# BlueFern/CRDModel

Measured on AMD Instinct MI355X. Metric: grid-point-steps/sec, FHN torus 8192x8192 RK4, higher is better.
Workload: dtype f64

## Files before the change

### crdmodel_amd/__init__.py

```python
from . import _capi
from ._capi import CrdError
from .solver import (Ensemble, LocalGroup, PinnedArray, Recorder, Slab, Writer, block_extents, cycle_agreed, cycle_vote, dims_create, grid_of, halo_plan, initial_conditions, kernel_digest, kernel_digest_of_table_row, kernel_table_digest, launch_plan_candidates, load_ini, make_params, plan_key, rccl_unique_id,
                     run_config, slab_extents, stable_dt, steady_state, steady_state_as_printed)
```

### crdmodel_amd/_capi.py

```python
import ctypes as C
import importlib.util
import os
import sys

_PKG = os.path.dirname(os.path.abspath(__file__))
LIB_PATH = os.environ.get("CRD_LIBRARY") or os.path.join(_PKG, "libcrd.so")

ABI_VERSION = 8
OK, EINVAL, ENOMEM, EHIP, ERCCL, EIO, EPARSE, ESTATE = 0, -1, -2, -3, -4, -5, -6, -7
MODEL_FHN, MODEL_GOLDBETER = 0, 1
SURFACE_TORUS, SURFACE_FLAT = 0, 1
PRECISION_F64, PRECISION_F32 = 0, 1
STEPPER_AUTO, STEPPER_STAGED, STEPPER_FUSED = 0, 1, 2
ADAPT_RK43, ADAPT_ARKODE = 0, 1

MODELS = {"fhn": MODEL_FHN, "goldbeter": MODEL_GOLDBETER}
SURFACES = {"torus": SURFACE_TORUS, "flat": SURFACE_FLAT}
STEPPERS = {"auto": STEPPER_AUTO, "staged": STEPPER_STAGED, "fused": STEPPER_FUSED}


class Params(C.Structure):

    _fields_ = [
        ("model", C.c_int32), ("surface", C.c_int32),
# ... 154 lines not shown
    "crd_dominant_kernel_name": (C.c_char_p, [_vp]),
    "crd_state_max_abs": (C.c_int, [_vp, C.POINTER(C.c_double)]),
    "crd_trace_range_push": (None, [C.c_char_p]),
    "crd_trace_range_pop": (None, []),
    "crd_set_autotune": (C.c_int, [_vp, C.c_int]),
    "crd_get_launch_plan": (C.c_int, [_vp, C.POINTER(LaunchPlan)]),
    "crd_get_launch_geometry": (C.c_int, [_vp, C.POINTER(LaunchGeometry)]),
    "crd_set_launch_plan": (C.c_int, [_vp, C.c_int, C.c_int, C.c_int, C.c_int, C.c_int]),
    "crd_plan_launches": (C.c_int, [_vp]),
    "crd_set_diagnostics": (C.c_int, [_vp, C.c_int]),
    "crd_set_halo_slack": (C.c_int, [_vp, C.c_int]),
    "crd_set_exchange_period": (C.c_int, [_vp, C.c_int]),
    "crd_get_exchange_period": (C.c_int, [_vp]),
    "crd_group_set_threads": (C.c_int, [C.POINTER(_vp), C.c_int, C.c_int]),
    "crd_launch_plan_candidate": (C.c_int, [C.c_int, C.POINTER(LaunchPlan)]),
    "crd_get_step_timing": (C.c_int, [_vp, C.POINTER(StepTiming)]),
    "crd_ensemble_create": (C.c_int, [C.POINTER(Params), C.c_int, C.c_int, C.POINTER(_vp)]),
    "crd_ensemble_create_mixed": (C.c_int, [C.POINTER(Params), C.c_int, C.c_int, C.POINTER(_vp)]),
    "crd_ensemble_member_grid": (C.c_int, [_vp, C.c_int, C.POINTER(Grid)]),
    "crd_ensemble_destroy": (None, [_vp]),
    "crd_ensemble_last_error": (C.c_char_p, [_vp]),
    "crd_ensemble_info": (C.c_int, [_vp, C.POINTER(C.c_int), C.POINTER(Grid)]),
    "crd_ensemble_upload": (C.c_int, [_vp, C.c_int, _vp, C.c_int]),
    "crd_ensemble_download": (C.c_int, [_vp, C.c_int, _vp, C.c_int]),
    "crd_ensemble_step_rk4": (C.c_int, [_vp, C.c_double, C.c_double, C.c_int64]),
    "crd_ensemble_step_rk4_own": (C.c_int, [_vp, C.c_double, C.c_double, C.POINTER(C.c_int64)]),
    "crd_ensemble_step_rk4_own_dt": (C.c_int, [_vp, C.c_double, C.c_double, C.POINTER(C.c_double), C.POINTER(C.c_int64)]),
    "crd_ensemble_step_rk4_own_timed": (C.c_int, [_vp, C.c_double, C.c_double, C.POINTER(C.c_int64), C.POINTER(C.c_double)]),
    "crd_ensemble_own_steps": (C.c_int, [_vp, C.c_double, C.c_double, C.c_double, C.POINTER(C.c_int64)]),
    "crd_ensemble_step_rk4_timed": (C.c_int, [_vp, C.c_double, C.c_double, C.c_int64, C.POINTER(C.c_double)]),
# ... 82 lines not shown
```

### crdmodel_amd/csrc/crd_context.cpp

```cpp
#include <algorithm>
#include <cmath>
#include <cstdio>
#include <cstdlib>
#include <cstring>
#include <new>

#include "crd_ctx.h"
#include "crd_ensemble.h"
#include "crd_tuning.h"

namespace crd {

namespace {
thread_local std::string g_create_error;
}

int fail(crd_ctx *c, int code, const std::string &msg)
{
	if (c) c->err = msg; else g_create_error = msg;
	return code;
}

int set_device(crd_ctx *c)
{
// ... 723 lines not shown
	hipDeviceProp_t prop;
	HIP_TRY(c, hipGetDeviceProperties(&prop, c->device));
	out->simds = 4 * prop.multiProcessorCount;
	out->clock_khz = prop.clockRate;
	return CRD_OK;
}

int crd_launch_plan_candidate(int index, crd_launch_plan *out)
{
	if (!out) return CRD_EINVAL;
	*out = crd_launch_plan{};
	if (!fused_plan_candidate(index, &out->one_round, &out->xcd_mapping, &out->columns_per_lane, &out->nontemporal_stores, &out->steps_per_launch)) return CRD_EINVAL;
	return CRD_OK;
}

int crd_state_max_abs(crd_ctx *c, double *out)
{
	if (!c || !out) return CRD_EINVAL;
	if (int rc = set_device(c)) return rc;
	double *sink = c->scalar_sink();
	HIP_TRY(c, launch_max_abs(c->p.precision, c->plane[crd_ctx::Y][0], c->nx, c->nyl, sink, c->compute));
	if (sink != c->scalar_host) HIP_TRY(c, hipMemcpyAsync(c->scalar_host, sink, sizeof(double), hipMemcpyDeviceToHost, c->compute));
	HIP_TRY(c, hipStreamSynchronize(c->compute));
	*out = c->scalar_host[0];
	return CRD_OK;
}

int crd_state_observe(crd_ctx *c, double stats[8])
{
	if (!c || !stats) return CRD_EINVAL;
// ... 57 lines not shown
```

### crdmodel_amd/csrc/crd_fused.hip

```cpp
#include "crd_fused_impl.h"

namespace crd {

bool fused_step_supported(int, const SlabDesc &d) { return d.nyl >= 2 * kStepHalo; }

bool fused_two_steps_supported(const SlabDesc &d) { return d.nyl >= 4 * kStepHalo && kernel_model(d) != kModelDiffusionOnly; }

int fused_steps_supported(int precision, const SlabDesc &d, int want)
{
	bool three = kernel_model(d) == CRD_MODEL_FHN && (precision == CRD_PRECISION_F64 || d.nx % 2 == 0);
#ifdef CRD_THREE_STEPS_GOLDBETER
	three = three || (precision == CRD_PRECISION_F64 && kernel_model(d) == CRD_MODEL_GOLDBETER);
#endif
	if (want >= 3 && three && (d.wrap || precision != CRD_PRECISION_F64) && d.nyl >= 6 * kStepHalo) return 3;
	return (want >= 2 && fused_two_steps_supported(d)) ? 2 : 1;
}

bool fused_wide_supported(int precision, const SlabDesc &d, int want_steps)
{
	return precision == CRD_PRECISION_F64 && kernel_model(d) == CRD_MODEL_FHN && fused_steps_supported(precision, d, want_steps) == 3;
}

int fused_max_items(const SlabDesc &d)
{
	const int strips = (d.nx + (kValid - 2) - 1) / (kValid - 2);
	return strips * ((d.nyl + 2 * kGhost + 3) / 4 + 2);
}

const char *fused_kernel_name(int, int) { return "crd_rk4_fused_step_kernel"; }

int fused_default_columns(int precision, int nx) { return (precision == CRD_PRECISION_F32 && nx % 2 == 0) ? 2 : 1; }
// ... 37 lines not shown
```

### crdmodel_amd/csrc/crd_fused_impl.h

```cpp
#pragma once
#include <hip/hip_runtime.h>
#include <hip/hip_ext.h>

#include <algorithm>
#include <cstdint>
#include <cstdio>
#include <cstdlib>
#include <type_traits>
#include <utility>

#include "crd_device.h"
#include "crd_tuning.h"

namespace crd {

namespace {

using namespace dev;

constexpr int kApron = 4;
constexpr int kLanes = 64;
constexpr int kValid = kLanes - 2 * kApron;
constexpr int kWavesPerBlock = 4;
constexpr int kMaxWavesPerBlock = 4;
// ... 81 lines not shown
template <typename Real, int MODEL, int COLS, int STEPS = 2>
constexpr bool kCoop = sizeof(Real) == 8 && COLS == 1;
#elif defined(CRD_NO_COOP)
template <typename Real, int MODEL, int COLS, int STEPS = 2>
constexpr bool kCoop = false;
#else
template <typename Real, int MODEL, int COLS, int STEPS = 2>
constexpr bool kCoop = sizeof(Real) == 8 && COLS == 1 && (MODEL == CRD_MODEL_GOLDBETER || STEPS == 3);
#endif
#if defined(CRD_NO_READ_AHEAD)
template <typename Real, int MODEL, int COLS, int STEPS>
constexpr bool kReadAhead = false;
#else
template <typename Real, int MODEL, int COLS, int STEPS>
constexpr bool kReadAhead = kCoop<Real, MODEL, COLS, STEPS> && STEPS == 3;
#endif
constexpr int kWideWaves = 8;
template <typename Real, int MODEL, int COLS, int STEPS>
constexpr bool kCanWide = sizeof(Real) == 8 && MODEL == CRD_MODEL_FHN && COLS == 1 && STEPS == 3 && kCoop<Real, MODEL, COLS, STEPS>;
template <int STEPS>
constexpr int kEdgeSlotBytes = STEPS == 3 ? 128 : 64;
template <int STEPS, int WAVES = 4 >
constexpr int kEdgeParityBytes = WAVES * 2 * kEdgeSlotBytes<STEPS>;
template <int STEPS, int WAVES = 4>
constexpr int kEdgeBytes = 2 * kEdgeParityBytes<STEPS, WAVES>;
template <int STEPS, int WAVES = 4>
constexpr int kEdgeDumpBytes = WAVES * 64 * 8 + kEdgeBytes<STEPS, WAVES>;
__device__ __forceinline__ double from_lane_below_old(double x, double old)
{
	int lo = __double2loint(x), hi = __double2hiint(x);
// ... 355 lines not shown
constexpr int kRingRowsWanted = CRD_RING_ROWS;
#ifndef CRD_RING_ROWS_THREE
#define CRD_RING_ROWS_THREE 8
#endif
template <typename V, int STEPS = 2>
constexpr int kRingRowsOf = (kLanes * (int)sizeof(V) / 256 >= 4 && (STEPS == 3 ? CRD_RING_ROWS_THREE : kRingRowsWanted) > 4) ? 4 : (STEPS == 3 ? CRD_RING_ROWS_THREE : kRingRowsWanted);
typedef unsigned int u32x2 __attribute__((ext_vector_type(2)));
typedef unsigned int u32x4 __attribute__((ext_vector_type(4)));
typedef __attribute__((address_space(3))) char lds_char;
constexpr unsigned kRowResourceBytes = 0x7fffffffu;
constexpr unsigned kStoreNowhere = 0x80000000u;
__device__ __forceinline__ __amdgpu_buffer_rsrc_t row_resource(const void *row)
{
	return __builtin_amdgcn_make_buffer_rsrc(const_cast<void *>(row), 0, (int)kRowResourceBytes, 0x00020000);
}
template <bool NT, typename V>
__device__ __forceinline__ void buffer_row_store(__amdgpu_buffer_rsrc_t r, unsigned byte_offset, V v)
{
	constexpr int aux = NT ? 2 : 0;
	if constexpr (sizeof(V) == 4) __builtin_amdgcn_raw_buffer_store_b32(__builtin_bit_cast(unsigned, v), r, byte_offset, 0, aux);
	else if constexpr (sizeof(V) == 8) __builtin_amdgcn_raw_buffer_store_b64(__builtin_bit_cast(u32x2, v), r, byte_offset, 0, aux);
	else __builtin_amdgcn_raw_buffer_store_b128(__builtin_bit_cast(u32x4, v), r, byte_offset, 0, aux);
}
template <int VMCNT, int OFF_U, int OFF_V, typename V>
__device__ __forceinline__ void ring_read(unsigned lds_lane, V &u, V &v)
{
	if constexpr (sizeof(V) == 4)
		asm volatile("s_waitcnt vmcnt(%3)\n\tds_read_b32 %0, %2 offset:%4\n\tds_read_b32 %1, %2 offset:%5\n\ts_waitcnt lgkmcnt(0)"
		             : "=&v"(u), "=&v"(v) : "v"(lds_lane), "n"(VMCNT), "n"(OFF_U), "n"(OFF_V) : "memory");
	else if constexpr (sizeof(V) == 8)
		asm volatile("s_waitcnt vmcnt(%3)\n\tds_read_b64 %0, %2 offset:%4\n\tds_read_b64 %1, %2 offset:%5\n\ts_waitcnt lgkmcnt(0)"
		             : "=&v"(u), "=&v"(v) : "v"(lds_lane), "n"(VMCNT), "n"(OFF_U), "n"(OFF_V) : "memory");
	else
		asm volatile("s_waitcnt vmcnt(%3)\n\tds_read_b128 %0, %2 offset:%4\n\tds_read_b128 %1, %2 offset:%5\n\ts_waitcnt lgkmcnt(0)"
		             : "=&v"(u), "=&v"(v) : "v"(lds_lane), "n"(VMCNT), "n"(OFF_U), "n"(OFF_V) : "memory");
}
template <int VMCNT, int OFF_U, int OFF_V>
// ... 58 lines not shown
#endif
#endif
	using V = typename LaneValue<Real, COLS>::type;
	constexpr int APRON = STEPS * kApron;
	constexpr int FILL = 2 * APRON;
	static_assert(APRON % COLS == 0, "the apron is whole lanes");
	constexpr int VALID = COLS * kLanes - 2 * APRON;
	constexpr int M = 4;
	constexpr int RB = kLanes * (int)sizeof(V), SLOT = 2 * RB, G1 = RB / 256, kRingRows = kRingRowsOf<V, STEPS>;
	static_assert(kRingRows % M == 0 && kRingRows >= M && (kRingRows & (kRingRows - 1)) == 0, "ring slots are addressed with the unrolled iteration index");
	constexpr int kWaitFill = (kRingRows - 1) * 2 * G1, kWaitSteady = kWaitFill + 2 * kRingRows;
	static_assert(kWaitSteady <= 63, "vmcnt is six bits");
	constexpr bool AHEAD = kReadAhead<Real, MODEL, COLS, STEPS>;
	constexpr int kWaitAhead = kWaitFill + 2 * (kRingRows - 1);
	static_assert(kWaitAhead <= 63, "vmcnt is six bits");
	const int lane = threadIdx.x & (kLanes - 1);
	const int nx = s.nx;
	const int wave = __builtin_amdgcn_readfirstlane((int)(threadIdx.x >> 6));
	const int x0 = COOP ? sblk * (a.sw * kLanes - 2 * APRON) - APRON + wave * kLanes : strip * VALID - APRON;
	const int place = COOP ? wave * kLanes + lane : COLS * lane, span = COOP ? a.sw * kLanes : COLS * kLanes;
	int x = x0 + COLS * lane;
	x %= nx;
	if (x < 0) x += nx;
	const unsigned xb = (unsigned)x * (unsigned)sizeof(Real);
	const int out_col = x0 + COLS * lane;
	const bool lane_stores = place >= APRON && place < span - APRON && out_col < nx;
	const unsigned xb_store = lane_stores ? xb : kStoreNowhere;

	const int range = chunk >= a.first2 ? 1 : 0;
	const int range_end = a.r_end[range];
// ... 1 lines not shown
	const int j1 = (j0 + a.chunk < range_end) ? j0 + a.chunk : range_end;
	const int jbase = j0 - APRON;
	const int niter = (j1 - j0) + 2 * APRON;
	const int jlast = j1 + APRON - 1;

	const V cE = *reinterpret_cast<const V *>(s.cE + x), cWn = *reinterpret_cast<const V *>(s.cWn + x), cP = *reinterpret_cast<const V *>(s.cP + x);
	const Real ka4 = s.ka4;
	const V h1 = (V)a.h1, h2 = (V)a.h2, h3 = (V)a.h3, h6 = (V)a.h6;
	const __attribute__((address_space(4))) Real *const brow = (const __attribute__((address_space(4))) Real *)(s.brow);
	const int wrap_nyl = s.wrap ? s.nyl : 0;
	auto row_base = [&](int j) -> ptrdiff_t {
		j += wrap_nyl & (j >> 31);
		j -= (j >= s.nyl) ? wrap_nyl : 0;
		return (ptrdiff_t)j * nx;
	};
	int jb = 0, amask = 0;
	if (ABSORB) {
		int g0 = (a.js + jbase) % a.ny;
		if (g0 < 0) g0 += a.ny;
		jb = jbase + (a.ny - 1 - g0);
#pragma unroll
		for (int k = 0; k < 4; k++) amask |= (a.absorb[k] ? 1 << k : 0) | (a.absorb2[k] ? 16 << k : 0) | ((STEPS == 3 && a.absorb3[k]) ? 256 << k : 0);
		jb = __builtin_amdgcn_readfirstlane(jb);
		amask = __builtin_amdgcn_readfirstlane(amask);
	}
	const int ny_rows = a.ny;
	auto boundary_row = [&](int j) -> bool { return (unsigned)(j - jb) <= 1u || (unsigned)(j - jb - ny_rows) <= 1u; };

	struct Pipe {
		V u0[M], v0[M], U1[M], U2[M], U3[M], V1[2], V2[2], V3[2], aU[M], aV[M];
// ... 16 lines not shown
	if constexpr (COOP) {
		const unsigned base = (unsigned)(uintptr_t)block_edges;
		edge_pub = (lane == 0 || lane == kLanes - 1) ? base + (unsigned)((wave * 2 + (lane == 0 ? 0 : 1)) * kEdgeSlotBytes<STEPS>)
		                                             : base + (unsigned)(kEdgeBytes<STEPS, WAVES> + (wave * kLanes + lane) * 8);
		edge_con = base + (unsigned)((lane == 0 ? (wave > 0 ? wave - 1 : wave) * 2 + 1 : (wave + 1 < a.sw ? wave + 1 : wave) * 2) * kEdgeSlotBytes<STEPS>);
	}
	const unsigned ring_lane = (unsigned)(uintptr_t)ring + (unsigned)lane * (unsigned)sizeof(V);
	unsigned doff[G1];
#pragma unroll
	for (int h = 0; h < G1; h++) {
		const int q = 4 * (kLanes * h + lane), e = q / (int)sizeof(Real);
		int col = (x0 + e) % nx;
		if (col < 0) col += nx;
		doff[h] = (unsigned)col * (unsigned)sizeof(Real) + (unsigned)(q % (int)sizeof(Real));
	}
	auto fill = [&](int jrow, int slot_byte) {
		const ptrdiff_t rb = row_base(jrow);
		const __amdgpu_buffer_rsrc_t ru = row_resource(a.in_u + rb), rv = row_resource(a.in_v + rb);
#pragma unroll
		for (int h = 0; h < G1; h++) __builtin_amdgcn_raw_ptr_buffer_load_lds(ru, ring + (slot_byte + 256 * h), 4, doff[h], 0, 0, 0);
#pragma unroll
		for (int h = 0; h < G1; h++) __builtin_amdgcn_raw_ptr_buffer_load_lds(rv, ring + (slot_byte + RB + 256 * h), 4, doff[h], 0, 0, 0);
	};
#pragma unroll
	for (int k = 0; k < kRingRows; k++) fill((jbase + k < jlast) ? jbase + k : jlast, k * SLOT);
	int jn = (jbase + kRingRows < jlast) ? jbase + kRingRows : jlast;
	if constexpr (AHEAD) ring_read_ahead<kWaitFill, 0, RB>(ring_lane, P[0].u0[0], P[0].v0[0]);
	Real pb = brow[jbase];
	int trip_byte = 0;
	unsigned ring_trip = ring_lane;
	Real *out_row_u = a.out_u + (ptrdiff_t)(jbase - APRON) * nx, *out_row_v = a.out_v + (ptrdiff_t)(jbase - APRON) * nx;
	if constexpr (AHEAD) ring_first_row_landed(P[0].u0[0], P[0].v0[0]);

	[[maybe_unused]] double2r edge[2 * STEPS];
#pragma unroll
	for (int q = 0; q < 2 * STEPS; q++) edge[q] = double2r{0.0, 0.0};
	auto point = [&](V uC, V uS, V uN, V v, Real rowp, bool zero, [[maybe_unused]] V X, V &du, V &dv) {
		if constexpr (COOP) rhs_lane_edge<MODEL>(uC, X, uS, uN, v, cE, cWn, cP, rowp, ka4, zero, du, dv);
		else rhs_lane<V, MODEL>(uC, uS, uN, v, cE, cWn, cP, rowp, ka4, zero, du, dv);
	};
	auto stages = [&](Pipe &Q, const int p, auto kk, auto live_c, const int flag_bit, const Real b4, V &nu, V &nv, [[maybe_unused]] const V (&E)[4], auto qbase_c) {
// ... 27 lines not shown
			Q.aV[S3] = stage_fma(h3, dv, Q.aV[S3]);
		}
		nu = nv = zero_v;
		if constexpr (live >= 8) {
			point(Q.U3[S4], Q.U3[S5], Q.U3[S3], Q.V3[S4 & 1], b4, ABSORB && ((amask >> (flag_bit + 3)) & 1) && boundary_row(p - 4), E[3], du, dv);
			nu = stage_fma(h6, du, Q.aU[S4]);
			nv = stage_fma(h6, dv, Q.aV[S4]);
		}
	};
	auto next_trip = [&]() {
		if constexpr (kRingRows > M) {
			trip_byte = (trip_byte + M * SLOT) & (kRingRows * SLOT - 1);
			ring_trip = ring_lane + (unsigned)trip_byte;
		}
	};
	auto iteration = [&](int m, auto kk, auto fed_c) {
		constexpr int FED = decltype(fed_c)::value;
		constexpr int K = decltype(kk)::value;
		constexpr int S0 = K % M, S4 = (K + 2 * M - 4) % M;
#if !defined(CRD_NO_LOCKSTEP) && !defined(CRD_NO_LOCKSTEP_TWO)
		if constexpr (sizeof(Real) == 4 && STEPS == 2) __builtin_amdgcn_s_barrier();
#endif
		const int p = jbase + m;
		Real b4[STEPS];
#pragma unroll
		for (int n = 0; n < STEPS; n++) b4[n] = P[n].bq[S4];
		if (!AHEAD && m < FILL + kRingRows) asm volatile("s_waitcnt vmcnt(%0)" ::"n"(kWaitFill) : "memory");
		V E[STEPS][4];
		auto take_row = [&]() {
			P[0].bq[S0] = uniform(pb);
#ifndef CRD_PROBE_NOLOAD
			fill(jn, trip_byte + S0 * SLOT);
#endif
			jn = (jn < jlast) ? jn + 1 : jlast;
		};
		if constexpr (AHEAD) {
			edge_publish<(K & 1) * kEdgeParityBytes<STEPS, WAVES>>(edge_pub, P[0].u0[S0]);
			take_row();
			if constexpr (K == M - 1) next_trip();
			ring_row_landed(edge);
			pb = brow[(p < jlast) ? p + 1 : jlast];
#pragma unroll
			for (int n = 0; n < STEPS; n++) E[n][0] = edge[2 * n].x, E[n][1] = edge[2 * n].y, E[n][2] = edge[2 * n + 1].x, E[n][3] = edge[2 * n + 1].y;
		} else if constexpr (COOP) {
			ring_read_with_edges<kWaitSteady, S0 * SLOT, S0 * SLOT + RB>(ring_trip, P[0].u0[S0], P[0].v0[S0], edge);
#pragma unroll
			for (int n = 0; n < STEPS; n++) E[n][0] = edge[2 * n].x, E[n][1] = edge[2 * n].y, E[n][2] = edge[2 * n + 1].x, E[n][3] = edge[2 * n + 1].y;
			edge_publish<(K & 1) * kEdgeParityBytes<STEPS, WAVES>>(edge_pub, P[0].u0[S0]);
		} else {
			ring_read<kWaitSteady, S0 * SLOT, S0 * SLOT + RB>(ring_trip, P[0].u0[S0], P[0].v0[S0]);
#pragma unroll
			for (int n = 0; n < STEPS; n++) E[n][0] = E[n][1] = E[n][2] = E[n][3] = zero_v;
		}
		if constexpr (!AHEAD) {
			take_row();
			pb = brow[(p < jlast) ? p + 1 : jlast];
		}
		V nu, nv;
		if constexpr (PRIO) __builtin_amdgcn_s_setprio(0);
		[[maybe_unused]] auto read_ahead = [&]() {
			if (m + 1 < FILL + kRingRows) asm volatile("s_waitcnt vmcnt(%0)" ::"n"(kWaitFill) : "memory");
			ring_read_ahead<kWaitAhead, ((K + 1) % M) * SLOT, ((K + 1) % M) * SLOT + RB>(ring_trip, P[0].u0[(K + 1) % M], P[0].v0[(K + 1) % M]);
		};
#ifdef CRD_PROBE_NOMATH
		nu = P[0].u0[S0] + (V)b4[0];
		nv = P[0].v0[S0] + (V)b4[STEPS - 1];
		if constexpr (AHEAD) read_ahead();
#else
		for_sequence(
		    [&](auto nn) {
			    constexpr int N = decltype(nn)::value;
#ifdef CRD_PROBE_HALFMATH
			    if constexpr (N > 0) return;
#endif
			    if constexpr (N > 0) {
				    P[N].u0[S0] = nu;
				    P[N].v0[S0] = nv;
				    P[N].bq[S0] = b4[N - 1];
				    if constexpr (COOP) edge_publish<(K & 1) * kEdgeParityBytes<STEPS, WAVES> + 32 * N>(edge_pub, nu);
			    }
			    constexpr int live = FED - 8 * N < 0 ? 0 : (FED - 8 * N > 8 ? 8 : FED - 8 * N);
			    stages(P[N], p - kApron * N, kk, std::integral_constant<int, live>{}, 4 * N, b4[N], nu, nv, E[N], std::integral_constant<int, 4 * N>{});
			    if constexpr (AHEAD && N == 0) read_ahead();
		    },
		    std::make_integer_sequence<int, STEPS>{});
#endif
		if constexpr (PRIO) __builtin_amdgcn_s_setprio(2);
		if constexpr (FED >= FILL) {
#if defined(CRD_PROBE_BRANCHY_STORES)
			if (lane_stores) {
				buffer_row_store<NT>(row_resource(out_row_u), xb, nu);
				buffer_row_store<NT>(row_resource(out_row_v), xb, nv);
			}
#elif !defined(CRD_PROBE_NOSTORE)
			buffer_row_store<NT>(row_resource(out_row_u), xb_store, nu);
			buffer_row_store<NT>(row_resource(out_row_v), xb_store, nv);
#else
			if (a.nchunks < 0) {
				buffer_row_store<NT>(row_resource(out_row_u), xb_store, nu);
				buffer_row_store<NT>(row_resource(out_row_v), xb_store, nv);
			}
#endif
		}
		out_row_u += nx;
		out_row_v += nx;
		if constexpr (AHEAD) edge_exchange<(K & 1) * kEdgeParityBytes<STEPS, WAVES>>(edge_con, edge, P[0].u0[(K + 1) % M], P[0].v0[(K + 1) % M]);
		else if constexpr (COOP) edge_exchange<(K & 1) * kEdgeParityBytes<STEPS, WAVES>>(edge_con, edge);
	};
	int m = 0;
	for_sequence(
	    [&](auto i) {
		    constexpr int I = decltype(i)::value;
		    iteration(I, std::integral_constant<int, I % M>{}, i);
		    if constexpr (!AHEAD && I % M == M - 1) next_trip();
	    },
	    std::make_integer_sequence<int, FILL>{});
	m = FILL;
	for (; m + M - 1 < niter; m += M) {
		for_sequence([&](auto k) { iteration(m + decltype(k)::value, k, std::integral_constant<int, FILL>{}); }, std::make_integer_sequence<int, M>{});
		if constexpr (!AHEAD) next_trip();
	}
	for_sequence(
	    [&](auto k) {
		    if (m + decltype(k)::value < niter) iteration(m + decltype(k)::value, k, std::integral_constant<int, FILL>{});
	    },
	    std::make_integer_sequence<int, M - 1>{});
	if constexpr (AHEAD)
		asm volatile("s_waitcnt vmcnt(0) lgkmcnt(0)"
		             : "+v"(P[0].u0[0]), "+v"(P[0].u0[1]), "+v"(P[0].u0[2]), "+v"(P[0].u0[3]), "+v"(P[0].v0[0]), "+v"(P[0].v0[1]), "+v"(P[0].v0[2]), "+v"(P[0].v0[3])
		             :
		             : "memory");
	else asm volatile("s_waitcnt vmcnt(0)" ::: "memory");
}

template <typename Real, int MODEL, int COLS, int STEPS, bool ABSORB>
constexpr int kMinWaves = (STEPS == 2 && COLS * (int)sizeof(Real) == 8 && MODEL == CRD_MODEL_FHN && !ABSORB) ? 3 : (STEPS == 3 ? 2 : 1);
template <typename Real, int MODEL, bool ABSORB, int EMBED, int COLS, bool NT = false, int STEPS = 1, int WAVES = kMaxWavesPerBlock>
__global__ void __launch_bounds__(kLanes *WAVES) __attribute__((amdgpu_waves_per_eu(kMinWaves<Real, MODEL, COLS, STEPS, ABSORB>))) crd_rk4_fused_step_kernel(Slab<Real> s, FusedArgs<Real> a)
{
// ... 157 lines not shown
hipError_t launch_fused_t(const SlabDesc &d, const FusedCall &c, int row_begin, int row_end, int row_begin2, int row_end2, int js, int ny,
                          hipStream_t st)
{
	clear_launch_status();
	if (row_end <= row_begin) {
		if (c.geometry) return hipSuccess;
		if (c.start_event)
			if (hipError_t e = hipEventRecord(c.start_event, st); e != hipSuccess) return e;
		if (c.done_event)
			if (hipError_t e = hipEventRecord(c.done_event, st); e != hipSuccess) return e;
		return hipSuccess;
	}
	if (row_end2 < row_begin2) row_end2 = row_begin2;
	constexpr bool kCanTwoSteps = MODEL != kModelDiffusionOnly;
	if (c.steps != 1 && (c.embed || !((c.steps == 2 && kCanTwoSteps) || (c.steps == 3 && kCanThreeSteps<Real, MODEL> && (kThreeStepCols<Real, MODEL> == 1 || d.nx % 2 == 0)))))
		return hipErrorInvalidValue;
	if (!d.wrap && (row_begin < -(kGhost - c.steps * kStepHalo) || row_end > d.nyl + (kGhost - c.steps * kStepHalo))) return hipErrorInvalidValue;
	const Slab<Real> s = typed<Real>(d);
	FusedArgs<Real> a;
	a.in_u = row0<Real>(c.y0.u, d.nx);
	a.in_v = row0<Real>(c.y0.v, d.nx);
	a.out_u = row0<Real>(c.yout.u, d.nx);
	a.out_v = row0<Real>(c.yout.v, d.nx);
	a.h2 = (Real)(0.5 * c.dt);
	a.h3 = (Real)(c.dt / 3.0);
	a.h6 = (Real)(c.dt / 6.0);
	a.h1 = (Real)c.dt;
	for (int k = 0; k < 5; k++) a.absorb[k] = c.absorb[k];
	for (int k = 0; k < 4; k++) a.absorb2[k] = c.absorb2[k];
	for (int k = 0; k < 4; k++) a.absorb3[k] = c.absorb3[k];
// ... 220 lines not shown
				else set_io(c.yout, c.tune_scratch);
				flip ^= 1;
			}
			return fire();
		};
		if (pingpong && err == hipSuccess) {
			configure(0, 0, cols_default, 0);
			err = fire();
		}
		constexpr int kCandidates = kNumPlanCandidates, kRounds = 3;
		const bool room_for_two = d.wrap || (row_begin >= -(kGhost - 2 * kStepHalo) && row_end <= d.nyl + (kGhost - 2 * kStepHalo));
		const bool two_steps_ok = kCanTwoSteps && !c.embed && c.steps == 1 && d.nyl >= 4 * kStepHalo && room_for_two;
		const bool room_for_three = d.wrap || (row_begin >= -(kGhost - 3 * kStepHalo) && row_end <= d.nyl + (kGhost - 3 * kStepHalo));
		const bool three_steps_ok = two_steps_ok && kCanThreeSteps<Real, MODEL> && (kThreeStepCols<Real, MODEL> == 1 || cols2_ok) && d.nyl >= 6 * kStepHalo &&
		                            (d.wrap || sizeof(Real) == 4) && room_for_three &&
		                            !(sizeof(Real) == 4 && absorb12);
		float t_best[kCandidates];
		bool live[kCandidates];
		int reps = 3;
		for (int k = 0; k < kCandidates; k++) {
			t_best[k] = 0.f;
			configure(kPlanCandidates[k].one_round, kPlanCandidates[k].remap, kPlanCandidates[k].cols, kPlanCandidates[k].nt, kPlanCandidates[k].steps);
			live[k] = k == 0 || !(kPlanCandidates[k].one_round && a.chunk == fused_chunk_rows<Real, MODEL>(a.nstrips, rows, 0, cols, steps));
			if (live[k] && kPlanCandidates[k].one_round != plan_mode) live[k] = false;
			if (live[k] && kPlanCandidates[k].steps != ((kPlanCandidates[k].steps == 3 ? three_steps_ok : two_steps_ok) ? steps : 1)) live[k] = false;
			if (live[k] && steps == 2 && cols == 2 && sizeof(Real) == 8) live[k] = false;
			if (live[k] && kPlanCandidates[k].remap != a.remap) live[k] = false;
			if (live[k] && kPlanCandidates[k].cols != cols) live[k] = false;
			if (live[k] && (kPlanCandidates[k].nt != 0) != nt) live[k] = false;
		}
// ... 112 lines not shown
```

### crdmodel_amd/csrc/crd_kernels.h

```cpp
#pragma once

#include <hip/hip_runtime.h>

#include <cstdint>

namespace crd {

struct Planes {
	void *u;
	void *v;
};

struct SlabDesc {
	const void *cE;
	const void *cWn;
	const void *cP;
	const void *brow;
	double ka4;
	int nx;
	int nyl;
	int wrap;
	int wrap_x = 1;
	int has_row0;
	int has_rowN;
// ... 67 lines not shown
	FusedGeometry *geometry = nullptr;
	hipEvent_t done_event = nullptr;
	hipEvent_t start_event = nullptr;
};
hipError_t launch_fused_step(int precision, const SlabDesc &d, const FusedCall &c, int row_begin, int row_end, int row_begin2, int row_end2,
                             hipStream_t s);
hipError_t launch_sum_partials(const double *partials, int n, double *out, hipEvent_t done, hipStream_t s);
const char *fused_kernel_name(int precision, int model);
bool fused_step_supported(int precision, const SlabDesc &d);
int fused_default_columns(int precision, int nx);
int fused_plan_candidates();
bool fused_plan_candidate(int index, int *chunk_mode, int *mapping, int *cols, int *nt, int *steps);
bool fused_two_steps_supported(const SlabDesc &d);
bool fused_wide_supported(int precision, const SlabDesc &d, int want_steps);
int fused_steps_supported(int precision, const SlabDesc &d, int want);
int fused_max_items(const SlabDesc &d);

hipError_t launch_aos_to_planes(int precision, int src_is_f64, const void *aos, Planes dst, int nx, int nyl, hipStream_t s);
hipError_t launch_planes_to_aos(int precision, int dst_is_f64, Planes src, void *aos, int nx, int nyl, hipStream_t s);
hipError_t launch_aos_row_extract(int precision, const void *aos, void *row, int nx, int j, hipStream_t s);
hipError_t launch_aos_cols_extract(int precision, const void *aos, void *col_w, void *col_e, int nx, int nyl, hipStream_t s);
hipError_t launch_plane_cols_extract(int precision, const void *u_plane, void *col_w, void *col_e, int nx, int nyl, hipStream_t s);

hipError_t launch_hermite(int precision, Planes yn, Planes yp, Planes fn, Planes fp, Planes out, int nx, int nyl, double theta, double h, hipStream_t s);

hipError_t launch_hin_bound(int precision, Planes y, Planes f, int nx, int nyl, double rtol, double atol, double *out_dev, hipStream_t s);
hipError_t launch_axpy_planes(int precision, Planes y, Planes f, double h, Planes out, int nx, int nyl, hipStream_t s);
hipError_t launch_ydd_sumsq(int precision, Planes y, Planes f0, Planes f2, double h, double rtol, double atol, int nx, int nyl, double *partials_dev, double *out_dev,
                            hipStream_t s);

// ... 6 lines not shown
```

### crdmodel_amd/solver.py

```python
import ctypes as C

import numpy as np

from . import _capi as capi
from .post import period_map
from ._capi import (MODELS, SURFACES, STEPPERS, PRECISION_F32, PRECISION_F64, CrdError, Grid, Params,
                    RunConfig, check, lib)


def make_params(model, surface, nx, surface_length, surface_width, diffusion, beta, *, ny=0, beta_min=0.0, beta_max=0.0,
                vary_beta=0, just_diffusion=0, t_boundary=0.0, precision="f64"):
    p = Params()
    p.model = MODELS[model] if isinstance(model, str) else model
    p.surface = SURFACES[surface] if isinstance(surface, str) else surface
    p.nx, p.ny = nx, ny
    p.surface_length, p.surface_width = surface_length, surface_width
    p.diffusion, p.beta, p.beta_min, p.beta_max = diffusion, beta, beta_min, beta_max
    p.vary_beta, p.just_diffusion = vary_beta, just_diffusion
    p.t_boundary = t_boundary
    p.precision = {"f64": PRECISION_F64, "f32": PRECISION_F32}[precision] if isinstance(precision, str) else precision
    return p


def grid_of(params):
# ... 556 lines not shown
        except Exception:
            pass


def launch_plan_candidates(eight_wide=False):
    out, k = [], 0
    while True:
        lp = capi.LaunchPlan()
        if lib().crd_launch_plan_candidate(k, C.byref(lp)) != 0:
            return out
        if (lp.one_round == 3) == bool(eight_wide):
            out.append((lp.one_round, lp.xcd_mapping, lp.columns_per_lane, lp.nontemporal_stores, lp.steps_per_launch))
        k += 1


def plan_key(model, precision, plan):
    if isinstance(plan, dict):
        plan = (plan["one_round"], plan["xcd_mapping"], plan["columns_per_lane"], plan["nontemporal_stores"], plan.get("steps_per_launch", 1))
    key = "fused/%s/%s/chunk%d/map%d/cols%d/%s" % (model, precision, plan[0], plan[1], plan[2], "nt" if plan[3] else "plain")
    return key + ("/steps%d" % plan[4] if len(plan) > 4 and plan[4] >= 2 else "")


def kernel_table_digest():
    return lib().crd_kernel_table_digest().decode()


def kernel_digest(geometry):
    import hashlib

    fields = ("vgprs", "sgprs", "lds_bytes", "scratch_bytes", "wavefronts_per_simd", "loop_valu", "loop_salu", "loop_vmem", "loop_lds", "loop_instructions", "exec_skipped_vmem")
# ... 188 lines not shown
```

### include/crd.h

```cpp
#ifndef CRD_H
#define CRD_H

#include <stddef.h>
#include <stdint.h>

#ifdef __cplusplus
extern "C" {
#endif

#define CRD_ABI_VERSION 8

typedef enum crd_status {
	CRD_OK = 0,
	CRD_EINVAL = -1,
	CRD_ENOMEM = -2,
	CRD_EHIP = -3,
	CRD_ERCCL = -4,
	CRD_EIO = -5,
	CRD_EPARSE = -6,
	CRD_ESTATE = -7
} crd_status;

enum { CRD_MODEL_FHN = 0, CRD_MODEL_GOLDBETER = 1 };
enum { CRD_SURFACE_TORUS = 0, CRD_SURFACE_FLAT = 1 };
// ... 221 lines not shown
	int32_t rows;
	int32_t strips, chunk_rows, chunks;
	int32_t workgroups, wavefronts_per_workgroup;
	int32_t fill_iterations;
	int32_t iterations_per_trip;
	int32_t lanes, lanes_valid;
	int32_t vgprs, sgprs, lds_bytes, scratch_bytes, wavefronts_per_simd;
	int32_t loop_valu, loop_salu, loop_vmem, loop_lds, loop_instructions;
	int32_t simds, clock_khz;
	int32_t exec_skipped_vmem;
	int64_t wavefront_iterations;
	int64_t wavefront_iterations_effective;
} crd_launch_geometry;
int crd_get_launch_geometry(crd_ctx *ctx, crd_launch_geometry *out);
int crd_launch_plan_candidate(int index, crd_launch_plan *out);
int crd_set_launch_plan(crd_ctx *ctx, int chunk_mode, int xcd_mapping, int columns_per_lane, int nontemporal_stores, int steps_per_launch);
int crd_plan_launches(crd_ctx *ctx);

void crd_trace_range_push(const char *name);
void crd_trace_range_pop(void);

int crd_state_max_abs(crd_ctx *ctx, double *out);

typedef struct crd_ensemble crd_ensemble;
int crd_ensemble_create(const crd_params *members, int n_members, int device, crd_ensemble **out);
int crd_ensemble_create_mixed(const crd_params *members, int n_members, int device, crd_ensemble **out);
void crd_ensemble_destroy(crd_ensemble *e);
const char *crd_ensemble_last_error(const crd_ensemble *e);
int crd_ensemble_info(const crd_ensemble *e, int *n_members, crd_grid *g);
int crd_ensemble_member_grid(const crd_ensemble *e, int member, crd_grid *g);
// ... 68 lines not shown
```

Measured before the change: 352.4 billion.

## Address fused three-step rows via scalar offsets on fixed buffer resources

In the read-ahead three-step fused kernel, per-row buffer resource construction for loads and stores is replaced. Four buffer resources are built once per slab, and a scalar row byte offset (soffset) is advanced each row, with a torus seam wrap. The steady-state loop is also peeled from the ring-fill phase so the conditional vmcnt wait drops out of the main loop. The aim is to cut scalar/vector address arithmetic and resource setup in the inner loop. A 32-bit addressability guard, with new C/Python query helpers, falls back to fewer steps per launch when a slab exceeds 4 GiB.

After: 358.7 billion, median of 6. +1.8%, better.

```diff
diff --git a/crdmodel_amd/__init__.py b/crdmodel_amd/__init__.py
--- a/crdmodel_amd/__init__.py
+++ b/crdmodel_amd/__init__.py
@@ -1,4 +1,4 @@
 from . import _capi
 from ._capi import CrdError
 from .solver import (Ensemble, LocalGroup, PinnedArray, Recorder, Slab, Writer, block_extents, cycle_agreed, cycle_vote, dims_create, grid_of, halo_plan, initial_conditions, kernel_digest, kernel_digest_of_table_row, kernel_table_digest, launch_plan_candidates, load_ini, make_params, plan_key, rccl_unique_id,
-                     run_config, slab_extents, stable_dt, steady_state, steady_state_as_printed)
+                     rows_addressable, run_config, slab_extents, stable_dt, steady_state, steady_state_as_printed, steps_per_launch_on)
diff --git a/crdmodel_amd/_capi.py b/crdmodel_amd/_capi.py
--- a/crdmodel_amd/_capi.py
+++ b/crdmodel_amd/_capi.py
@@ -192,6 +192,8 @@
     "crd_get_exchange_period": (C.c_int, [_vp]),
     "crd_group_set_threads": (C.c_int, [C.POINTER(_vp), C.c_int, C.c_int]),
     "crd_launch_plan_candidate": (C.c_int, [C.c_int, C.POINTER(LaunchPlan)]),
+    "crd_steps_per_launch_on": (C.c_int, [C.c_int, C.c_int, C.c_int64, C.c_int64, C.c_int, C.c_int]),
+    "crd_rows_addressable": (C.c_int, [C.c_int64, C.c_int64, C.c_int]),
     "crd_get_step_timing": (C.c_int, [_vp, C.POINTER(StepTiming)]),
     "crd_ensemble_create": (C.c_int, [C.POINTER(Params), C.c_int, C.c_int, C.POINTER(_vp)]),
     "crd_ensemble_create_mixed": (C.c_int, [C.POINTER(Params), C.c_int, C.c_int, C.POINTER(_vp)]),
diff --git a/crdmodel_amd/csrc/crd_context.cpp b/crdmodel_amd/csrc/crd_context.cpp
--- a/crdmodel_amd/csrc/crd_context.cpp
+++ b/crdmodel_amd/csrc/crd_context.cpp
@@ -761,6 +761,26 @@
 	return CRD_OK;
 }
 
+int crd_rows_addressable(int64_t nx, int64_t rows, int real_bytes)
+{
+	if (nx > INT32_MAX || rows > INT32_MAX) return 0;
+	return fused_scalar_rows_addressable((long)nx, (long)rows, (long)real_bytes) ? 1 : 0;
+}
+
+int crd_steps_per_launch_on(int model, int precision, int64_t nx, int64_t nyl, int single_slab, int steps_wanted)
+{
+	if ((model != CRD_MODEL_FHN && model != CRD_MODEL_GOLDBETER) || (precision != CRD_PRECISION_F64 && precision != CRD_PRECISION_F32) || nx < 1 || nyl < 1 || nx > INT32_MAX ||
+	    nyl > INT32_MAX || steps_wanted < 1 || steps_wanted > 3)
+		return CRD_EINVAL;
+	SlabDesc d{};
+	d.nx = (int)nx;
+	d.nyl = (int)nyl;
+	d.ny = (int)nyl;
+	d.wrap = single_slab ? 1 : 0;
+	d.model = model;
+	return fused_steps_supported(precision, d, steps_wanted);
+}
+
 int crd_state_max_abs(crd_ctx *c, double *out)
 {
 	if (!c || !out) return CRD_EINVAL;
diff --git a/crdmodel_amd/csrc/crd_fused.hip b/crdmodel_amd/csrc/crd_fused.hip
--- a/crdmodel_amd/csrc/crd_fused.hip
+++ b/crdmodel_amd/csrc/crd_fused.hip
@@ -12,9 +12,12 @@
 #ifdef CRD_THREE_STEPS_GOLDBETER
 	three = three || (precision == CRD_PRECISION_F64 && kernel_model(d) == CRD_MODEL_GOLDBETER);
 #endif
+	if (precision == CRD_PRECISION_F64 && !fused_scalar_rows_addressable(d.nx, fused_addressed_rows(d), 8)) three = false;
 	if (want >= 3 && three && (d.wrap || precision != CRD_PRECISION_F64) && d.nyl >= 6 * kStepHalo) return 3;
 	return (want >= 2 && fused_two_steps_supported(d)) ? 2 : 1;
 }
+
+long fused_addressed_rows(const SlabDesc &d) { return (long)d.nyl + (d.wrap ? 0L : 2L * kGhost); }
 
 bool fused_wide_supported(int precision, const SlabDesc &d, int want_steps)
 {
diff --git a/crdmodel_amd/csrc/crd_fused_impl.h b/crdmodel_amd/csrc/crd_fused_impl.h
--- a/crdmodel_amd/csrc/crd_fused_impl.h
+++ b/crdmodel_amd/csrc/crd_fused_impl.h
@@ -119,6 +119,13 @@
 #else
 template <typename Real, int MODEL, int COLS, int STEPS>
 constexpr bool kReadAhead = kCoop<Real, MODEL, COLS, STEPS> && STEPS == 3;
+#endif
+#if defined(CRD_NO_SCALAR_ROWS)
+template <typename Real, int MODEL, int COLS, int STEPS>
+constexpr bool kScalarRows = false;
+#else
+template <typename Real, int MODEL, int COLS, int STEPS>
+constexpr bool kScalarRows = kReadAhead<Real, MODEL, COLS, STEPS>;
 #endif
 constexpr int kWideWaves = 8;
 template <typename Real, int MODEL, int COLS, int STEPS>
@@ -504,13 +511,23 @@
 {
 	return __builtin_amdgcn_make_buffer_rsrc(const_cast<void *>(row), 0, (int)kRowResourceBytes, 0x00020000);
 }
+template <bool ON>
+struct ScalarRows {
+};
+template <>
+struct ScalarRows<true> {
+	__amdgpu_buffer_rsrc_t in_u, in_v, out_u, out_v;
+	unsigned pitch, seam, in_off, out_off, b_off, b_last;
+	int row_lo;
+	const __attribute__((address_space(4))) char *b_first;
+};
 template <bool NT, typename V>
-__device__ __forceinline__ void buffer_row_store(__amdgpu_buffer_rsrc_t r, unsigned byte_offset, V v)
+__device__ __forceinline__ void buffer_row_store(__amdgpu_buffer_rsrc_t r, unsigned byte_offset, V v, unsigned row_offset = 0)
 {
 	constexpr int aux = NT ? 2 : 0;
-	if constexpr (sizeof(V) == 4) __builtin_amdgcn_raw_buffer_store_b32(__builtin_bit_cast(unsigned, v), r, byte_offset, 0, aux);
-	else if constexpr (sizeof(V) == 8) __builtin_amdgcn_raw_buffer_store_b64(__builtin_bit_cast(u32x2, v), r, byte_offset, 0, aux);
-	else __builtin_amdgcn_raw_buffer_store_b128(__builtin_bit_cast(u32x4, v), r, byte_offset, 0, aux);
+	if constexpr (sizeof(V) == 4) __builtin_amdgcn_raw_buffer_store_b32(__builtin_bit_cast(unsigned, v), r, byte_offset, row_offset, aux);
+	else if constexpr (sizeof(V) == 8) __builtin_amdgcn_raw_buffer_store_b64(__builtin_bit_cast(u32x2, v), r, byte_offset, row_offset, aux);
+	else __builtin_amdgcn_raw_buffer_store_b128(__builtin_bit_cast(u32x4, v), r, byte_offset, row_offset, aux);
 }
 template <int VMCNT, int OFF_U, int OFF_V, typename V>
 __device__ __forceinline__ void ring_read(unsigned lds_lane, V &u, V &v)
@@ -599,6 +616,8 @@
 	constexpr bool AHEAD = kReadAhead<Real, MODEL, COLS, STEPS>;
 	constexpr int kWaitAhead = kWaitFill + 2 * (kRingRows - 1);
 	static_assert(kWaitAhead <= 63, "vmcnt is six bits");
+	constexpr bool SROWS = kScalarRows<Real, MODEL, COLS, STEPS>;
+	static_assert(!SROWS || AHEAD, "scalar row offsets: the read-ahead block strip");
 	const int lane = threadIdx.x & (kLanes - 1);
 	const int nx = s.nx;
 	const int wave = __builtin_amdgcn_readfirstlane((int)(threadIdx.x >> 6));
@@ -630,6 +649,22 @@
 		j -= (j >= s.nyl) ? wrap_nyl : 0;
 		return (ptrdiff_t)j * nx;
 	};
+	[[maybe_unused]] ScalarRows<SROWS> sr;
+	[[maybe_unused]] auto row_offset = [&](int j, auto &rows) -> unsigned {
+		j += wrap_nyl & (j >> 31);
+		j -= (j >= s.nyl) ? wrap_nyl : 0;
+		return (unsigned)(j - rows.row_lo) * rows.pitch;
+	};
+	if constexpr (SROWS) {
+		sr.pitch = (unsigned)nx * (unsigned)sizeof(Real);
+		sr.row_lo = s.wrap ? 0 : -kGhost;
+		sr.seam = s.wrap ? (unsigned)s.nyl * sr.pitch : 0xffffffffu;
+		const ptrdiff_t lo = (ptrdiff_t)sr.row_lo * nx;
+		sr.in_u = row_resource(a.in_u + lo);
+		sr.in_v = row_resource(a.in_v + lo);
+		sr.out_u = row_resource(a.out_u + lo);
+		sr.out_v = row_resource(a.out_v + lo);
+	}
 	int jb = 0, amask = 0;
 	if (ABSORB) {
 		int g0 = (a.js + jbase) % a.ny;
@@ -676,17 +711,34 @@
 		if (col < 0) col += nx;
 		doff[h] = (unsigned)col * (unsigned)sizeof(Real) + (unsigned)(q % (int)sizeof(Real));
 	}
+	[[maybe_unused]] auto fill_from = [&](const auto ru, const auto rv, unsigned row_off, int slot_byte) {
+#pragma unroll
+		for (int h = 0; h < G1; h++) __builtin_amdgcn_raw_ptr_buffer_load_lds(ru, ring + (slot_byte + 256 * h), 4, doff[h], row_off, 0, 0);
+#pragma unroll
+		for (int h = 0; h < G1; h++) __builtin_amdgcn_raw_ptr_buffer_load_lds(rv, ring + (slot_byte + RB + 256 * h), 4, doff[h], row_off, 0, 0);
+	};
 	auto fill = [&](int jrow, int slot_byte) {
-		const ptrdiff_t rb = row_base(jrow);
-		const __amdgpu_buffer_rsrc_t ru = row_resource(a.in_u + rb), rv = row_resource(a.in_v + rb);
-#pragma unroll
-		for (int h = 0; h < G1; h++) __builtin_amdgcn_raw_ptr_buffer_load_lds(ru, ring + (slot_byte + 256 * h), 4, doff[h], 0, 0, 0);
-#pragma unroll
-		for (int h = 0; h < G1; h++) __builtin_amdgcn_raw_ptr_buffer_load_lds(rv, ring + (slot_byte + RB + 256 * h), 4, doff[h], 0, 0, 0);
+		if constexpr (SROWS) {
+			fill_from(sr.in_u, sr.in_v, row_offset(jrow, sr), slot_byte);
+		} else {
+			const ptrdiff_t rb = row_base(jrow);
+			const __amdgpu_buffer_rsrc_t ru = row_resource(a.in_u + rb), rv = row_resource(a.in_v + rb);
+#pragma unroll
+			for (int h = 0; h < G1; h++) __builtin_amdgcn_raw_ptr_buffer_load_lds(ru, ring + (slot_byte + 256 * h), 4, doff[h], 0, 0, 0);
+#pragma unroll
+			for (int h = 0; h < G1; h++) __builtin_amdgcn_raw_ptr_buffer_load_lds(rv, ring + (slot_byte + RB + 256 * h), 4, doff[h], 0, 0, 0);
+		}
 	};
 #pragma unroll
 	for (int k = 0; k < kRingRows; k++) fill((jbase + k < jlast) ? jbase + k : jlast, k * SLOT);
 	int jn = (jbase + kRingRows < jlast) ? jbase + kRingRows : jlast;
+	if constexpr (SROWS) {
+		sr.in_off = row_offset(jn, sr);
+		sr.out_off = (unsigned)(jbase - APRON - sr.row_lo) * sr.pitch;
+		sr.b_first = (const __attribute__((address_space(4))) char *)(brow + jbase);
+		sr.b_off = 0;
+		sr.b_last = (unsigned)(jlast - jbase) * (unsigned)sizeof(Real);
+	}
 	if constexpr (AHEAD) ring_read_ahead<kWaitFill, 0, RB>(ring_lane, P[0].u0[0], P[0].v0[0]);
 	Real pb = brow[jbase];
 	int trip_byte = 0;
@@ -744,8 +796,9 @@
 			ring_trip = ring_lane + (unsigned)trip_byte;
 		}
 	};
-	auto iteration = [&](int m, auto kk, auto fed_c) {
+	auto iteration = [&](int m, auto kk, auto fed_c, auto steady_c) {
 		constexpr int FED = decltype(fed_c)::value;
+		constexpr bool STEADY = decltype(steady_c)::value;
 		constexpr int K = decltype(kk)::value;
 		constexpr int S0 = K % M, S4 = (K + 2 * M - 4) % M;
 #if !defined(CRD_NO_LOCKSTEP) && !defined(CRD_NO_LOCKSTEP_TWO)
@@ -760,16 +813,29 @@
 		auto take_row = [&]() {
 			P[0].bq[S0] = uniform(pb);
 #ifndef CRD_PROBE_NOLOAD
-			fill(jn, trip_byte + S0 * SLOT);
-#endif
+			if constexpr (SROWS) fill_from(sr.in_u, sr.in_v, sr.in_off, trip_byte + S0 * SLOT);
+			else fill(jn, trip_byte + S0 * SLOT);
+#endif
+			if constexpr (SROWS) {
+				sr.in_off += (jn < jlast) ? sr.pitch : 0u;
+				sr.in_off = (sr.in_off == sr.seam) ? 0u : sr.in_off;
+			}
 			jn = (jn < jlast) ? jn + 1 : jlast;
+		};
+		[[maybe_unused]] auto next_b = [&]() {
+			if constexpr (SROWS) {
+				sr.b_off = (sr.b_off + (unsigned)sizeof(Real) < sr.b_last) ? sr.b_off + (unsigned)sizeof(Real) : sr.b_last;
+				pb = *(const __attribute__((address_space(4))) Real *)(sr.b_first + sr.b_off);
+			} else {
+				pb = brow[(p < jlast) ? p + 1 : jlast];
+			}
 		};
 		if constexpr (AHEAD) {
 			edge_publish<(K & 1) * kEdgeParityBytes<STEPS, WAVES>>(edge_pub, P[0].u0[S0]);
 			take_row();
 			if constexpr (K == M - 1) next_trip();
 			ring_row_landed(edge);
-			pb = brow[(p < jlast) ? p + 1 : jlast];
+			next_b();
 #pragma unroll
 			for (int n = 0; n < STEPS; n++) E[n][0] = edge[2 * n].x, E[n][1] = edge[2 * n].y, E[n][2] = edge[2 * n + 1].x, E[n][3] = edge[2 * n + 1].y;
 		} else if constexpr (COOP) {
@@ -789,7 +855,8 @@
 		V nu, nv;
 		if constexpr (PRIO) __builtin_amdgcn_s_setprio(0);
 		[[maybe_unused]] auto read_ahead = [&]() {
-			if (m + 1 < FILL + kRingRows) asm volatile("s_waitcnt vmcnt(%0)" ::"n"(kWaitFill) : "memory");
+			if constexpr (!STEADY)
+				if (m + 1 < FILL + kRingRows) asm volatile("s_waitcnt vmcnt(%0)" ::"n"(kWaitFill) : "memory");
 			ring_read_ahead<kWaitAhead, ((K + 1) % M) * SLOT, ((K + 1) % M) * SLOT + RB>(ring_trip, P[0].u0[(K + 1) % M], P[0].v0[(K + 1) % M]);
 		};
 #ifdef CRD_PROBE_NOMATH
@@ -818,13 +885,19 @@
 		if constexpr (PRIO) __builtin_amdgcn_s_setprio(2);
 		if constexpr (FED >= FILL) {
 #if defined(CRD_PROBE_BRANCHY_STORES)
+			static_assert(!SROWS, "the probe stores through the row pointers: build it with -DCRD_NO_SCALAR_ROWS");
 			if (lane_stores) {
 				buffer_row_store<NT>(row_resource(out_row_u), xb, nu);
 				buffer_row_store<NT>(row_resource(out_row_v), xb, nv);
 			}
 #elif !defined(CRD_PROBE_NOSTORE)
-			buffer_row_store<NT>(row_resource(out_row_u), xb_store, nu);
-			buffer_row_store<NT>(row_resource(out_row_v), xb_store, nv);
+			if constexpr (SROWS) {
+				buffer_row_store<NT>(sr.out_u, xb_store, nu, sr.out_off);
+				buffer_row_store<NT>(sr.out_v, xb_store, nv, sr.out_off);
+			} else {
+				buffer_row_store<NT>(row_resource(out_row_u), xb_store, nu);
+				buffer_row_store<NT>(row_resource(out_row_v), xb_store, nv);
+			}
 #else
 			if (a.nchunks < 0) {
 				buffer_row_store<NT>(row_resource(out_row_u), xb_store, nu);
@@ -832,8 +905,12 @@
 			}
 #endif
 		}
-		out_row_u += nx;
-		out_row_v += nx;
+		if constexpr (SROWS) {
+			sr.out_off += sr.pitch;
+		} else {
+			out_row_u += nx;
+			out_row_v += nx;
+		}
 		if constexpr (AHEAD) edge_exchange<(K & 1) * kEdgeParityBytes<STEPS, WAVES>>(edge_con, edge, P[0].u0[(K + 1) % M], P[0].v0[(K + 1) % M]);
 		else if constexpr (COOP) edge_exchange<(K & 1) * kEdgeParityBytes<STEPS, WAVES>>(edge_con, edge);
 	};
@@ -841,18 +918,34 @@
 	for_sequence(
 	    [&](auto i) {
 		    constexpr int I = decltype(i)::value;
-		    iteration(I, std::integral_constant<int, I % M>{}, i);
+		    iteration(I, std::integral_constant<int, I % M>{}, i, std::false_type{});
 		    if constexpr (!AHEAD && I % M == M - 1) next_trip();
 	    },
 	    std::make_integer_sequence<int, FILL>{});
 	m = FILL;
-	for (; m + M - 1 < niter; m += M) {
-		for_sequence([&](auto k) { iteration(m + decltype(k)::value, k, std::integral_constant<int, FILL>{}); }, std::make_integer_sequence<int, M>{});
-		if constexpr (!AHEAD) next_trip();
+	if constexpr (SROWS) {
+		bool whole = true;
+		for_sequence(
+		    [&](auto t) {
+			    constexpr int M0 = FILL + M * decltype(t)::value;
+			    whole = whole && M0 + M - 1 < niter;
+			    if (whole) {
+				    for_sequence([&](auto k) { iteration(M0 + decltype(k)::value, k, std::integral_constant<int, FILL>{}, std::false_type{}); }, std::make_integer_sequence<int, M>{});
+				    m = M0 + M;
+			    }
+		    },
+		    std::make_integer_sequence<int, kRingRows / M>{});
+		for (; m + M - 1 < niter; m += M)
+			for_sequence([&](auto k) { iteration(m + decltype(k)::value, k, std::integral_constant<int, FILL>{}, std::true_type{}); }, std::make_integer_sequence<int, M>{});
+	} else {
+		for (; m + M - 1 < niter; m += M) {
+			for_sequence([&](auto k) { iteration(m + decltype(k)::value, k, std::integral_constant<int, FILL>{}, std::false_type{}); }, std::make_integer_sequence<int, M>{});
+			if constexpr (!AHEAD) next_trip();
+		}
 	}
 	for_sequence(
 	    [&](auto k) {
-		    if (m + decltype(k)::value < niter) iteration(m + decltype(k)::value, k, std::integral_constant<int, FILL>{});
+		    if (m + decltype(k)::value < niter) iteration(m + decltype(k)::value, k, std::integral_constant<int, FILL>{}, std::false_type{});
 	    },
 	    std::make_integer_sequence<int, M - 1>{});
 	if constexpr (AHEAD)
@@ -1040,6 +1133,8 @@
 	if (row_end2 < row_begin2) row_end2 = row_begin2;
 	constexpr bool kCanTwoSteps = MODEL != kModelDiffusionOnly;
 	if (c.steps != 1 && (c.embed || !((c.steps == 2 && kCanTwoSteps) || (c.steps == 3 && kCanThreeSteps<Real, MODEL> && (kThreeStepCols<Real, MODEL> == 1 || d.nx % 2 == 0)))))
+		return hipErrorInvalidValue;
+	if (c.steps == 3 && kScalarRows<Real, MODEL, kThreeStepCols<Real, MODEL>, 3> && !fused_scalar_rows_addressable(d.nx, fused_addressed_rows(d), (long)sizeof(Real)))
 		return hipErrorInvalidValue;
 	if (!d.wrap && (row_begin < -(kGhost - c.steps * kStepHalo) || row_end > d.nyl + (kGhost - c.steps * kStepHalo))) return hipErrorInvalidValue;
 	const Slab<Real> s = typed<Real>(d);
@@ -1290,6 +1385,7 @@
 		const bool room_for_three = d.wrap || (row_begin >= -(kGhost - 3 * kStepHalo) && row_end <= d.nyl + (kGhost - 3 * kStepHalo));
 		const bool three_steps_ok = two_steps_ok && kCanThreeSteps<Real, MODEL> && (kThreeStepCols<Real, MODEL> == 1 || cols2_ok) && d.nyl >= 6 * kStepHalo &&
 		                            (d.wrap || sizeof(Real) == 4) && room_for_three &&
+		                            (!kScalarRows<Real, MODEL, kThreeStepCols<Real, MODEL>, 3> || fused_scalar_rows_addressable(d.nx, fused_addressed_rows(d), (long)sizeof(Real))) &&
 		                            !(sizeof(Real) == 4 && absorb12);
 		float t_best[kCandidates];
 		bool live[kCandidates];
diff --git a/crdmodel_amd/csrc/crd_kernels.h b/crdmodel_amd/csrc/crd_kernels.h
--- a/crdmodel_amd/csrc/crd_kernels.h
+++ b/crdmodel_amd/csrc/crd_kernels.h
@@ -105,6 +105,13 @@
 bool fused_two_steps_supported(const SlabDesc &d);
 bool fused_wide_supported(int precision, const SlabDesc &d, int want_steps);
 int fused_steps_supported(int precision, const SlabDesc &d, int want);
+inline bool fused_scalar_rows_addressable(long nx, long rows, long real_bytes)
+{
+	if (nx < 1 || rows < 1 || real_bytes < 1) return false;
+	const unsigned long pitch = (unsigned long)nx * (unsigned long)real_bytes, limit = 1ul << 32;
+	return pitch < limit && (unsigned long)rows <= limit / pitch && (unsigned long)rows * pitch < limit - pitch;
+}
+long fused_addressed_rows(const SlabDesc &d);
 int fused_max_items(const SlabDesc &d);
 
 hipError_t launch_aos_to_planes(int precision, int src_is_f64, const void *aos, Planes dst, int nx, int nyl, hipStream_t s);
diff --git a/crdmodel_amd/solver.py b/crdmodel_amd/solver.py
--- a/crdmodel_amd/solver.py
+++ b/crdmodel_amd/solver.py
@@ -594,6 +594,18 @@
         k += 1
 
 
+def steps_per_launch_on(model, precision, nx, nyl, steps_wanted, single_slab=True):
+    rc = lib().crd_steps_per_launch_on(MODELS[model] if isinstance(model, str) else model,
+                                       {"f64": PRECISION_F64, "f32": PRECISION_F32}[precision] if isinstance(precision, str) else precision,
+                                       nx, nyl, 1 if single_slab else 0, steps_wanted)
+    check(min(rc, 0), "crd_steps_per_launch_on")
+    return rc
+
+
+def rows_addressable(nx, rows, real_bytes=8):
+    return bool(lib().crd_rows_addressable(nx, rows, real_bytes))
+
+
 def plan_key(model, precision, plan):
     if isinstance(plan, dict):
         plan = (plan["one_round"], plan["xcd_mapping"], plan["columns_per_lane"], plan["nontemporal_stores"], plan.get("steps_per_launch", 1))
diff --git a/include/crd.h b/include/crd.h
--- a/include/crd.h
+++ b/include/crd.h
@@ -259,6 +259,8 @@
 } crd_launch_geometry;
 int crd_get_launch_geometry(crd_ctx *ctx, crd_launch_geometry *out);
 int crd_launch_plan_candidate(int index, crd_launch_plan *out);
+int crd_steps_per_launch_on(int model, int precision, int64_t nx, int64_t nyl, int single_slab, int steps_wanted);
+int crd_rows_addressable(int64_t nx, int64_t rows, int real_bytes);
 int crd_set_launch_plan(crd_ctx *ctx, int chunk_mode, int xcd_mapping, int columns_per_lane, int nontemporal_stores, int steps_per_launch);
 int crd_plan_launches(crd_ctx *ctx);
 
```
